# wangrui2025/GDKVM

Hardware: AMD Instinct MI355X
Metric: frames/sec (GDKVM forward + argmax mask), EchoNet 112x112x32 clips (higher is better)
Workload: dtype bf16; 1 GPU; BASELINE.json configs[1]: EchoNet-Dynamic 112x112x32 bf16 inference, batch=16 per GPU; clips_per_gpu=16, frames_per_clip=32, image=112x112, heads=1, key_dim=64, rule=delta_sequential, world_size=1, ranks_seen=1

## Files before the change

### gdkvm_amd/csrc/conv_igemm.hip

```cpp
#include <atomic>

#include "gdkvm_device.hpp"

namespace {

constexpr int IG_TN = 128;
constexpr int IG_WAVES_N = 4;
constexpr int IG_GD = 2;

struct IgArgs {
    const bf16_t* x; const bf16_t* w; const float* bias; const bf16_t* res; bf16_t* y;
    int N, H, W, C, K, R, S, stride, pad, Ho, Wo, relu;
    int M, ksteps, cps;
    const bf16_t* w2; const float* bias2; bf16_t* y2; int centre;
    float inv_cps, inv_s;
    struct Cls { const bf16_t* w; int S, ksteps_main, ksteps_all, ksteps_row; float inv_s; } cls[4];
    const bf16_t* x2; int OH, OW;
};

template <int TM, int SUB, int TN = IG_TN, int WN = IG_WAVES_N, bool DG = false>
__global__ __launch_bounds__(256, 2) void conv_igemm_kernel(IgArgs a)
{
    constexpr int NTW = TN / 16 / WN;
    constexpr int MT = TM / 16 / (4 / WN);
    constexpr int PITCH = SUB == 2 ? 160 : 80;
    constexpr int PPP = 4 * SUB;
    constexpr int GP = TM * PPP / 256;
    constexpr int WD = SUB == 2 ? 2 : 3;
    constexpr int UF = SUB == 2 ? 2 : 6;
    __shared__ __attribute__((aligned(16))) unsigned char s_a[2][TM * PITCH];
    const int tid = threadIdx.x, lane = tid & 63, li = lane & 15, g = lane >> 4;
    const int w = __builtin_amdgcn_readfirstlane(tid >> 6), wm = w / WN, wn = w % WN;
    const int m0 = blockIdx.x * TM, n0 = blockIdx.y * TN;
    const int cls = DG ? (int)blockIdx.z : 0;
    const int S_ = DG ? a.cls[cls].S : a.S;
    const float inv_s_ = DG ? a.cls[cls].inv_s : a.inv_s;
    const int nsteps = (DG ? a.cls[cls].ksteps_all : a.ksteps) / SUB;
    const int main_steps = DG ? a.cls[cls].ksteps_main / SUB : nsteps;
    const ptrdiff_t x2_diff = DG && a.x2 ? a.x2 - a.x : 0;

    int g_iy0[GP], g_ix0[GP];
    const bf16_t* g_base[GP];
    unsigned g_lds[GP];
#pragma unroll
    for (int u = 0; u < GP; ++u) {
        const int q = 256 * u + tid, px = q / PPP, part = q % PPP;
        const int gp = min(m0 + px, a.M - 1);
        const int gn = gp / (a.Ho * a.Wo), grem = gp - gn * a.Ho * a.Wo, gyo = grem / a.Wo, gxo = grem - gyo * a.Wo;
        g_iy0[u] = m0 + px < a.M ? gyo * a.stride - a.pad : -0x40000000;
        g_ix0[u] = gxo * a.stride - a.pad;
        g_base[u] = a.x + (size_t)gn * a.H * a.W * a.C + 8 * part;
        g_lds[u] = (unsigned)(px * PITCH + 16 * part);
    }
    uint4 ga[IG_GD][GP];
    unsigned gok[IG_GD];
    const int spt = a.cps / SUB;
    const float inv_spt = a.inv_cps * (float)SUB;
    auto gather = [&](int st, uint4 (&d)[GP], unsigned& okm) __attribute__((always_inline)) {
        const bool second = DG && st >= main_steps;
        const int stm = second ? st - main_steps : st;
        const int tap = idx_div(stm, inv_spt), c0 = (stm - tap * spt) * 32 * SUB, r = idx_div(tap, inv_s_), s = tap - r * S_;
        const ptrdiff_t src = second ? x2_diff : 0;
        okm = 0;
#pragma unroll
        for (int u = 0; u < GP; ++u) {
            const int iy = g_iy0[u] + r, ix = g_ix0[u] + s;
            const bool ok = (unsigned)iy < (unsigned)a.H && (unsigned)ix < (unsigned)a.W;
            okm |= ok ? 1u << u : 0u;
            d[u] = *reinterpret_cast<const uint4*>(g_base[u] + src + ((size_t)(ok ? iy : 0) * a.W + (ok ? ix : 0)) * a.C + c0);
        }
    };
    auto put = [&](int buf, const uint4 (&d)[GP], unsigned okm) __attribute__((always_inline)) {
#pragma unroll
        for (int u = 0; u < GP; ++u) {
            const unsigned m = (okm >> u) & 1u ? 0xffffffffu : 0u;
            *reinterpret_cast<uint4*>(&s_a[buf][g_lds[u]]) = make_uint4(d[u].x & m, d[u].y & m, d[u].z & m, d[u].w & m);
        }
    };

    const unsigned abase = (unsigned)((16 * MT * wm + li) * PITCH + 16 * g);

    auto run_pass = [&](const bf16_t* wpk, int g0, int L, const float* bias, const bf16_t* res, bf16_t* y, int relu, int Lrow) __attribute__((always_inline)) {
        const bf16_t* wp = wpk + ((size_t)((n0 + 16 * NTW * wn) / 16) * (Lrow * SUB) * 64 + lane) * 8;
        const size_t nt_stride = (size_t)(Lrow * SUB) * 512;
        bf16x8 wr[WD][SUB][NTW];
        auto wload = [&](int l, bf16x8 (&d)[SUB][NTW]) __attribute__((always_inline)) {
            const size_t off = (size_t)min(l, L - 1) * (512 * SUB);
#pragma unroll
            for (int sb = 0; sb < SUB; ++sb)
#pragma unroll
                for (int nt = 0; nt < NTW; ++nt) d[sb][nt] = *reinterpret_cast<const bf16x8*>(wp + nt * nt_stride + off + 512 * sb);
        };
        const int glast = g0 + L - 1;
        f32x4 acc[MT][NTW];
#pragma unroll
        for (int mt = 0; mt < MT; ++mt)
#pragma unroll
            for (int nt = 0; nt < NTW; ++nt) acc[mt][nt] = f32x4{0.f, 0.f, 0.f, 0.f};

        gather(min(g0, glast), ga[0], gok[0]);
        gather(min(g0 + 1, glast), ga[1], gok[1]);
#pragma unroll
        for (int d = 0; d < WD; ++d) wload(d, wr[d]);
        put(0, ga[0], gok[0]);
        gather(min(g0 + 2, glast), ga[0], gok[0]);
        __syncthreads();

        auto step = [&](int l, auto jc) __attribute__((always_inline)) {
            constexpr int j = decltype(jc)::value % WD, gs = (decltype(jc)::value + 1) & 1;
            const int buf = l & 1;
#pragma unroll
            for (int sb = 0; sb < SUB; ++sb)
#pragma unroll
                for (int mt = 0; mt < MT; ++mt) {
                    const bf16x8 xa = *reinterpret_cast<const bf16x8*>(&s_a[buf][abase + mt * 16 * PITCH + 64 * sb]);
#pragma unroll
                    for (int nt = 0; nt < NTW; ++nt) acc[mt][nt] = __builtin_amdgcn_mfma_f32_16x16x32_bf16(wr[j][sb][nt], xa, acc[mt][nt], 0, 0, 0);
                }
            put(buf ^ 1, ga[gs], gok[gs]);
            wload(l + WD, wr[j]);
            gather(min(g0 + l + 1 + IG_GD, glast), ga[gs], gok[gs]);
            __syncthreads();
        };
        int l = 0;
        for (; l + UF <= L; l += UF)
            static_for<0, UF>([&](auto jc) { step(l + decltype(jc)::value, jc); });
        static_for<0, UF - 1>([&](auto jc) { if (l + decltype(jc)::value < L) step(l + decltype(jc)::value, jc); });

        const float lo = relu ? 0.f : -INFINITY;
#pragma unroll
        for (int nt = 0; nt < NTW; ++nt) {
            const int ch = n0 + 16 * NTW * wn + 16 * nt + 4 * g;
            const f32x4 b4 = bias ? *reinterpret_cast<const f32x4*>(bias + ch) : f32x4{0.f, 0.f, 0.f, 0.f};
#pragma unroll
            for (int mt = 0; mt < MT; ++mt) {
                const int p = m0 + 16 * MT * wm + 16 * mt + li;
                if (p >= a.M) continue;
                f32x4 v = acc[mt][nt] + b4;
                size_t o = (size_t)p * a.K + ch;
                if constexpr (DG) {
                    const int pn = p / (a.Ho * a.Wo), prem = p - pn * a.Ho * a.Wo, ya = prem / a.Wo, xb = prem - ya * a.Wo;
                    const int oy = 2 * ya + (cls >> 1), ox = 2 * xb + (cls & 1);
                    if (oy >= a.OH || ox >= a.OW) continue;
                    o = (((size_t)pn * a.OH + oy) * a.OW + ox) * a.K + ch;
                }
                if (res) {
                    const uint2 rr = *reinterpret_cast<const uint2*>(res + o);
                    v[0] += bf16_lo(rr.x); v[1] += bf16_hi(rr.x);
                    v[2] += bf16_lo(rr.y); v[3] += bf16_hi(rr.y);
                }
#pragma unroll
                for (int r = 0; r < 4; ++r) v[r] = fmaxf(v[r], lo);
                *reinterpret_cast<uint2*>(y + o) = make_uint2(pack_bf16x2(v[0], v[1]), pack_bf16x2(v[2], v[3]));
            }
        }
    };
    if constexpr (DG) {
        run_pass(a.cls[cls].w, 0, nsteps, nullptr, nullptr, a.y, 0, a.cls[cls].ksteps_row / SUB);
    } else {
        run_pass(a.w, 0, nsteps, a.bias, a.res, a.y, a.relu, nsteps);
        if (a.w2) run_pass(a.w2, a.centre * spt, spt, a.bias2, nullptr, a.y2, 0, spt);
    }
}

__global__ __launch_bounds__(256) void conv_igemm_pack_kernel(const uint4* w, uint4* packed, int K, int Kd)
{
    const int nks = Kd / 32;
    const size_t total = (size_t)(K / 16) * nks * 64;
    for (size_t i = (size_t)blockIdx.x * 256 + threadIdx.x; i < total; i += (size_t)gridDim.x * 256) {
        const int lane = (int)(i & 63), li = lane & 15, g = lane >> 4;
        const size_t f = i >> 6;
        const int ks = (int)(f % nks), nt = (int)(f / nks);
        packed[i] = w[((size_t)(16 * nt + li) * Kd + 32 * ks + 8 * g) / 8];
    }
}

}

extern "C" int gdkvm_conv_igemm_pack_weights(const void* w, void* packed, int K, int C, int R, int S, int io_dtype, void* stream)
{
    if (io_dtype != GDKVM_BF16) return gdkvm_fail(GDKVM_ERR_DTYPE, "conv_igemm_pack_weights: only bf16 is implemented");
    if (K <= 0 || C <= 0 || R <= 0 || S <= 0 || K % 16 || C % 32)
        return gdkvm_fail(GDKVM_ERR_SHAPE, "conv_igemm_pack_weights: K=%d C=%d %dx%d (K a multiple of 16, C of 32)", K, C, R, S);
    if (!w || !packed || !gdkvm_aligned16(w) || !gdkvm_aligned16(packed)) return gdkvm_fail(GDKVM_ERR_ARG, "conv_igemm_pack_weights: null or unaligned pointer");
    if (int rc = gdkvm_check_device()) return rc;
    const int Kd = R * S * C;
    const size_t total = (size_t)(K / 16) * (Kd / 32) * 64;
    hipLaunchKernelGGL(conv_igemm_pack_kernel, dim3((unsigned)((total + 255) / 256 > 4096 ? 4096 : (total + 255) / 256)), dim3(256), 0,
                       static_cast<hipStream_t>(stream), static_cast<const uint4*>(w), static_cast<uint4*>(packed), K, Kd);
    GDKVM_LAUNCH_CHECK("conv_igemm_pack_kernel");
    return GDKVM_OK;
}

int gdkvm_conv_igemm_launch(const void* x, const void* wpacked, const float* bias, const void* residual, void* y,
                            int N, int C, int H, int W, int K, int R, int S, int stride, int pad, int relu,
                            const void* w2packed, const float* bias2, void* y2, hipStream_t st)
{
    if (C % 32 || K % IG_TN || N < 1 || R < 1 || S < 1 || stride < 1 || pad < 0) return 1;
    if (w2packed && (!y2 || R != S || !(R & 1) || pad != R / 2)) return 1;
    const int Ho = (H + 2 * pad - R) / stride + 1, Wo = (W + 2 * pad - S) / stride + 1;
    if (Ho < 1 || Wo < 1) return 1;
    const long long M = (long long)N * Ho * Wo;
    if (M * (long long)(K > C ? K : C) > 0x7fffffffLL || (long long)N * H * W * C > 0x7fffffffLL || (long long)R * S * C / 32 > 65535) return 1;
    IgArgs a{};
    a.x = static_cast<const bf16_t*>(x); a.w = static_cast<const bf16_t*>(wpacked); a.bias = bias;
    a.res = static_cast<const bf16_t*>(residual); a.y = static_cast<bf16_t*>(y);
    a.w2 = static_cast<const bf16_t*>(w2packed); a.bias2 = bias2; a.y2 = static_cast<bf16_t*>(y2); a.centre = (R / 2) * S + S / 2;
    a.N = N; a.H = H; a.W = W; a.C = C; a.K = K; a.R = R; a.S = S; a.stride = stride; a.pad = pad; a.Ho = Ho; a.Wo = Wo; a.relu = relu;
    a.M = (int)M; a.cps = C / 32; a.ksteps = R * S * a.cps;
    a.inv_cps = 1.0f / (float)a.cps; a.inv_s = 1.0f / (float)S;
    const dim3 grid((unsigned)((M + 127) / 128), (unsigned)(K / IG_TN));
    if (C % 64 == 0) hipLaunchKernelGGL((conv_igemm_kernel<128, 2>), grid, dim3(256), 0, st, a);
    else hipLaunchKernelGGL((conv_igemm_kernel<128, 1>), grid, dim3(256), 0, st, a);
    return 0;
}

int gdkvm_conv_igemm_dgrad_launch(const void* dy, const void* dy2, const void* packs, int with_down, void* dx, int N, int Cf, int H, int W, int Kf, hipStream_t st)
{
    if (Cf % 64 || Kf % 64 || N < 1 || H < 1 || W < 1) return 1;
    const int Ho = (H - 1) / 2 + 1, Wo = (W - 1) / 2 + 1;
    const long long M = (long long)N * Ho * Wo;
    if (M * Kf > 0x7fffffffLL || (long long)N * H * W * Cf > 0x7fffffffLL || 5LL * Kf / 32 > 65535) return 1;
    IgArgs a{};
    a.x = static_cast<const bf16_t*>(dy); a.x2 = static_cast<const bf16_t*>(dy2); a.y = static_cast<bf16_t*>(dx);
    a.N = N; a.H = Ho; a.W = Wo; a.C = Kf; a.K = Cf; a.R = 1; a.S = 1; a.stride = 1; a.pad = 0; a.Ho = Ho; a.Wo = Wo; a.relu = 0;
    a.OH = H; a.OW = W;
    a.M = (int)M; a.cps = Kf / 32; a.ksteps = a.cps;
    a.inv_cps = 1.0f / (float)a.cps; a.inv_s = 1.0f;
    const bf16_t* wp = static_cast<const bf16_t*>(packs);
    for (int c = 0; c < 4; ++c) {
        const int ph = c >> 1, pw = c & 1, taps = (1 + ph) * (1 + pw);
        a.cls[c].w = wp;
        a.cls[c].S = 1 + pw;
        a.cls[c].inv_s = 1.0f / (float)(1 + pw);
        a.cls[c].ksteps_main = taps * a.cps;
        a.cls[c].ksteps_all = (taps + (c == 0 && dy2 && with_down ? 1 : 0)) * a.cps;
        a.cls[c].ksteps_row = (taps + (c == 0 && with_down ? 1 : 0)) * a.cps;
        wp += gdkvm_conv_s2_dgrad_pack_elems(Cf, Kf, c, with_down);
    }
    if (Cf % 128 == 0) {
        const dim3 grid((unsigned)((M + 127) / 128), (unsigned)(Cf / 128), 4);
        hipLaunchKernelGGL((conv_igemm_kernel<128, 2, 128, 4, true>), grid, dim3(256), 0, st, a);
    } else {
        const dim3 grid((unsigned)((M + 127) / 128), (unsigned)(Cf / 64), 4);
        hipLaunchKernelGGL((conv_igemm_kernel<128, 2, 64, 2, true>), grid, dim3(256), 0, st, a);
    }
    return 0;
}
```

Measured before the change: 681,600 frames/s.

## Pipeline conv igemm loads with inline asm and explicit vmcnt waits

Replaces the compiler-generated global loads in the implicit-GEMM conv kernel with inline-asm global_load_dwordx4 and counted s_waitcnt vmcnt waits. Each step now waits only for the specific weight or gather set it consumes, so later prefetches stay in flight. __syncthreads is replaced by lgkmcnt(0)+s_barrier, and the prologue is rewritten as earlier steps of the same schedule. The aim is to stop the compiler from inserting conservative vmcnt(0) waits that serialize memory and MFMA. The risk is that wrong counts or register naming give silent data hazards, and the code is fragile to changes in GP and NW.

```diff
diff --git a/gdkvm_amd/csrc/conv_igemm.hip b/gdkvm_amd/csrc/conv_igemm.hip
--- a/gdkvm_amd/csrc/conv_igemm.hip
+++ b/gdkvm_amd/csrc/conv_igemm.hip
@@ -52,11 +52,15 @@
         g_base[u] = a.x + (size_t)gn * a.H * a.W * a.C + 8 * part;
         g_lds[u] = (unsigned)(px * PITCH + 16 * part);
     }
-    uint4 ga[IG_GD][GP];
+    constexpr int NW = SUB * NTW;
+    static_assert(GP == NW && (GP == 2 || GP == 4), "gwait / wwait / drain name two or four registers per set");
+    static_assert(UF % WD == 0 && UF % 2 == 0 && WD <= IG_GD + 1, "the prologue is the steps -(IG_GD + 1) .. -1 of the same schedule");
+    u32x4 ga[IG_GD][GP];
     unsigned gok[IG_GD];
+    bf16x8 wr[WD][SUB][NTW];
     const int spt = a.cps / SUB;
     const float inv_spt = a.inv_cps * (float)SUB;
-    auto gather = [&](int st, uint4 (&d)[GP], unsigned& okm) __attribute__((always_inline)) {
+    auto gather = [&](int st, u32x4 (&d)[GP], unsigned& okm) __attribute__((always_inline)) {
         const bool second = DG && st >= main_steps;
         const int stm = second ? st - main_steps : st;
         const int tap = idx_div(stm, inv_spt), c0 = (stm - tap * spt) * 32 * SUB, r = idx_div(tap, inv_s_), s = tap - r * S_;
@@ -67,48 +71,57 @@
             const int iy = g_iy0[u] + r, ix = g_ix0[u] + s;
             const bool ok = (unsigned)iy < (unsigned)a.H && (unsigned)ix < (unsigned)a.W;
             okm |= ok ? 1u << u : 0u;
-            d[u] = *reinterpret_cast<const uint4*>(g_base[u] + src + ((size_t)(ok ? iy : 0) * a.W + (ok ? ix : 0)) * a.C + c0);
-        }
-    };
-    auto put = [&](int buf, const uint4 (&d)[GP], unsigned okm) __attribute__((always_inline)) {
+            const bf16_t* gp = g_base[u] + src + ((size_t)(ok ? iy : 0) * a.W + (ok ? ix : 0)) * a.C + c0;
+            asm volatile("global_load_dwordx4 %0, %1, off" : "=&v"(d[u]) : "v"(gp) : "memory");
+        }
+    };
+    auto gwait = [&](u32x4 (&d)[GP], auto nc) __attribute__((always_inline)) {
+        constexpr int N = decltype(nc)::value;
+        if constexpr (GP == 2) asm volatile("s_waitcnt vmcnt(%2)" : "+v"(d[0]), "+v"(d[1]) : "n"(N) : "memory");
+        else asm volatile("s_waitcnt vmcnt(%4)" : "+v"(d[0]), "+v"(d[1]), "+v"(d[2]), "+v"(d[3]) : "n"(N) : "memory");
+    };
+    auto wwait = [&](bf16x8 (&d)[SUB][NTW], auto nc) __attribute__((always_inline)) {
+        constexpr int N = decltype(nc)::value;
+        if constexpr (NW == 2) asm volatile("s_waitcnt vmcnt(%2)" : "+v"(d[0][0]), "+v"(d[0][1]) : "n"(N) : "memory");
+        else asm volatile("s_waitcnt vmcnt(%4)" : "+v"(d[0][0]), "+v"(d[0][1]), "+v"(d[SUB - 1][0]), "+v"(d[SUB - 1][1]) : "n"(N) : "memory");
+    };
+    auto put = [&](int buf, const u32x4 (&d)[GP], unsigned okm) __attribute__((always_inline)) {
 #pragma unroll
         for (int u = 0; u < GP; ++u) {
             const unsigned m = (okm >> u) & 1u ? 0xffffffffu : 0u;
-            *reinterpret_cast<uint4*>(&s_a[buf][g_lds[u]]) = make_uint4(d[u].x & m, d[u].y & m, d[u].z & m, d[u].w & m);
-        }
+            *reinterpret_cast<uint4*>(&s_a[buf][g_lds[u]]) = make_uint4(d[u][0] & m, d[u][1] & m, d[u][2] & m, d[u][3] & m);
+        }
+    };
+    auto barrier = [&]() __attribute__((always_inline)) {
+        asm volatile("s_waitcnt lgkmcnt(0)" ::: "memory");
+        asm volatile("s_barrier" ::: "memory");
     };
 
     const unsigned abase = (unsigned)((16 * MT * wm + li) * PITCH + 16 * g);
 
-    auto run_pass = [&](const bf16_t* wpk, int g0, int L, const float* bias, const bf16_t* res, bf16_t* y, int relu, int Lrow) __attribute__((always_inline)) {
-        const bf16_t* wp = wpk + ((size_t)((n0 + 16 * NTW * wn) / 16) * (Lrow * SUB) * 64 + lane) * 8;
-        const size_t nt_stride = (size_t)(Lrow * SUB) * 512;
-        bf16x8 wr[WD][SUB][NTW];
-        auto wload = [&](int l, bf16x8 (&d)[SUB][NTW]) __attribute__((always_inline)) {
-            const size_t off = (size_t)min(l, L - 1) * (512 * SUB);
-#pragma unroll
-            for (int sb = 0; sb < SUB; ++sb)
-#pragma unroll
-                for (int nt = 0; nt < NTW; ++nt) d[sb][nt] = *reinterpret_cast<const bf16x8*>(wp + nt * nt_stride + off + 512 * sb);
-        };
-        const int glast = g0 + L - 1;
-        f32x4 acc[MT][NTW];
-#pragma unroll
-        for (int mt = 0; mt < MT; ++mt)
-#pragma unroll
-            for (int nt = 0; nt < NTW; ++nt) acc[mt][nt] = f32x4{0.f, 0.f, 0.f, 0.f};
-
-        gather(min(g0, glast), ga[0], gok[0]);
-        gather(min(g0 + 1, glast), ga[1], gok[1]);
-#pragma unroll
-        for (int d = 0; d < WD; ++d) wload(d, wr[d]);
-        put(0, ga[0], gok[0]);
-        gather(min(g0 + 2, glast), ga[0], gok[0]);
-        __syncthreads();
-
-        auto step = [&](int l, auto jc) __attribute__((always_inline)) {
-            constexpr int j = decltype(jc)::value % WD, gs = (decltype(jc)::value + 1) & 1;
-            const int buf = l & 1;
+    struct Pass { const bf16_t* wrow[NTW]; int g0, L, glast; };
+    auto open_pass = [&](const bf16_t* wpk, int g0, int L, int Lrow) __attribute__((always_inline)) {
+        Pass p;
+#pragma unroll
+        for (int nt = 0; nt < NTW; ++nt) p.wrow[nt] = wpk + ((size_t)((n0 + 16 * NTW * wn) / 16 + nt) * (Lrow * SUB) * 64 + lane) * 8;
+        p.g0 = g0; p.L = L; p.glast = g0 + L - 1;
+        return p;
+    };
+    auto wload = [&](const Pass& p, int l, bf16x8 (&d)[SUB][NTW]) __attribute__((always_inline)) {
+        const size_t off = (size_t)min(l, p.L - 1) * (512 * SUB);
+#pragma unroll
+        for (int sb = 0; sb < SUB; ++sb)
+#pragma unroll
+            for (int nt = 0; nt < NTW; ++nt) asm volatile("global_load_dwordx4 %0, %1, off" : "=&v"(d[sb][nt]) : "v"(p.wrow[nt] + off + 512 * sb) : "memory");
+    };
+    f32x4 acc[MT][NTW];
+
+    constexpr int CW = GP + (WD - 1) * (GP + NW), CG = (IG_GD - 1) * (GP + NW);
+    auto step = [&](const Pass& p, int l, auto jc, auto mf) __attribute__((always_inline)) {
+        constexpr int j = decltype(jc)::value % WD, gs = (decltype(jc)::value + 1) & 1;
+        const int buf = l & 1;
+        if constexpr (decltype(mf)::value) {
+            wwait(wr[j], std::integral_constant<int, CW>{});
 #pragma unroll
             for (int sb = 0; sb < SUB; ++sb)
 #pragma unroll
@@ -117,29 +130,57 @@
 #pragma unroll
                     for (int nt = 0; nt < NTW; ++nt) acc[mt][nt] = __builtin_amdgcn_mfma_f32_16x16x32_bf16(wr[j][sb][nt], xa, acc[mt][nt], 0, 0, 0);
                 }
-            put(buf ^ 1, ga[gs], gok[gs]);
-            wload(l + WD, wr[j]);
-            gather(min(g0 + l + 1 + IG_GD, glast), ga[gs], gok[gs]);
-            __syncthreads();
-        };
+        }
+        gwait(ga[gs], std::integral_constant<int, CG>{});
+        put(buf ^ 1, ga[gs], gok[gs]);
+        wload(p, l + WD, wr[j]);
+        gather(min(p.g0 + l + 1 + IG_GD, p.glast), ga[gs], gok[gs]);
+        barrier();
+    };
+    auto request = [&](const Pass& p) __attribute__((always_inline)) {
+        static_for<0, IG_GD>([&](auto sc) {
+            constexpr int s = decltype(sc)::value - (IG_GD + 1);
+            if constexpr (s + WD >= 0) wload(p, s + WD, wr[(s + WD) % WD]);
+            gather(min(p.g0 + s + 1 + IG_GD, p.glast), ga[(s + 1 + IG_GD) & 1], gok[(s + 1 + IG_GD) & 1]);
+        });
+    };
+    auto run_pass = [&](const Pass& p, const float* bias, const bf16_t* res, bf16_t* y, int relu) __attribute__((always_inline)) {
+#pragma unroll
+        for (int mt = 0; mt < MT; ++mt)
+#pragma unroll
+            for (int nt = 0; nt < NTW; ++nt) acc[mt][nt] = f32x4{0.f, 0.f, 0.f, 0.f};
+        request(p);
+        step(p, -1, std::integral_constant<int, UF - 1>{}, std::false_type{});
         int l = 0;
-        for (; l + UF <= L; l += UF)
-            static_for<0, UF>([&](auto jc) { step(l + decltype(jc)::value, jc); });
-        static_for<0, UF - 1>([&](auto jc) { if (l + decltype(jc)::value < L) step(l + decltype(jc)::value, jc); });
-
-        const float lo = relu ? 0.f : -INFINITY;
+        for (; l + UF <= p.L; l += UF)
+            static_for<0, UF>([&](auto jc) { step(p, l + decltype(jc)::value, jc, std::true_type{}); });
+        static_for<0, UF - 1>([&](auto jc) { if (l + decltype(jc)::value < p.L) step(p, l + decltype(jc)::value, jc, std::true_type{}); });
+
+        f32x4 b4[NTW];
 #pragma unroll
         for (int nt = 0; nt < NTW; ++nt) {
             const int ch = n0 + 16 * NTW * wn + 16 * nt + 4 * g;
-            const f32x4 b4 = bias ? *reinterpret_cast<const f32x4*>(bias + ch) : f32x4{0.f, 0.f, 0.f, 0.f};
+            if (bias) asm volatile("global_load_dwordx4 %0, %1, off" : "=&v"(b4[nt]) : "v"(bias + ch) : "memory");
+            else b4[nt] = f32x4{0.f, 0.f, 0.f, 0.f};
+        }
+        asm volatile("s_waitcnt vmcnt(0)" : "+v"(b4[0]), "+v"(b4[1]) :: "memory");
+#pragma unroll
+        for (int d = 0; d < IG_GD; ++d) gwait(ga[d], std::integral_constant<int, 0>{});
+#pragma unroll
+        for (int d = 0; d < WD; ++d) wwait(wr[d], std::integral_constant<int, 0>{});
+
+        const float lo = relu ? 0.f : -INFINITY;
+#pragma unroll
+        for (int nt = 0; nt < NTW; ++nt) {
+            const int ch = n0 + 16 * NTW * wn + 16 * nt + 4 * g;
 #pragma unroll
             for (int mt = 0; mt < MT; ++mt) {
-                const int p = m0 + 16 * MT * wm + 16 * mt + li;
-                if (p >= a.M) continue;
-                f32x4 v = acc[mt][nt] + b4;
-                size_t o = (size_t)p * a.K + ch;
+                const int p_ = m0 + 16 * MT * wm + 16 * mt + li;
+                if (p_ >= a.M) continue;
+                f32x4 v = acc[mt][nt] + b4[nt];
+                size_t o = (size_t)p_ * a.K + ch;
                 if constexpr (DG) {
-                    const int pn = p / (a.Ho * a.Wo), prem = p - pn * a.Ho * a.Wo, ya = prem / a.Wo, xb = prem - ya * a.Wo;
+                    const int pn = p_ / (a.Ho * a.Wo), prem = p_ - pn * a.Ho * a.Wo, ya = prem / a.Wo, xb = prem - ya * a.Wo;
                     const int oy = 2 * ya + (cls >> 1), ox = 2 * xb + (cls & 1);
                     if (oy >= a.OH || ox >= a.OW) continue;
                     o = (((size_t)pn * a.OH + oy) * a.OW + ox) * a.K + ch;
@@ -156,10 +197,11 @@
         }
     };
     if constexpr (DG) {
-        run_pass(a.cls[cls].w, 0, nsteps, nullptr, nullptr, a.y, 0, a.cls[cls].ksteps_row / SUB);
+        const Pass p = open_pass(a.cls[cls].w, 0, nsteps, a.cls[cls].ksteps_row / SUB);
+        run_pass(p, nullptr, nullptr, a.y, 0);
     } else {
-        run_pass(a.w, 0, nsteps, a.bias, a.res, a.y, a.relu, nsteps);
-        if (a.w2) run_pass(a.w2, a.centre * spt, spt, a.bias2, nullptr, a.y2, 0, spt);
+        run_pass(open_pass(a.w, 0, nsteps, nsteps), a.bias, a.res, a.y, a.relu);
+        if (a.w2) run_pass(open_pass(a.w2, a.centre * spt, spt, spt), a.bias2, nullptr, a.y2, 0);
     }
 }
 
```

Measured after the change: 686,800 frames/s, median of 6. About the same (+0.8%).
